# BachiLi/redner

Measured on AMD Instinct MI355X. Metric: Msamples/s fwd+bwd, higher is better.
Workload: dtype f64; 1 GPU; bunny_box 1024x1024, max_bounces 4, Sobol, 256 spp fwd+bwd per step (vertex gradients, primary+secondary edge sampling), sharded by sample index over 1 GPU(s): 256 spp per GPU; spp=256, spp_per_gpu=256, max_bounces=4, parallelism=sample-sharded x1, world_size=1, pool_cap_mb=32768, samples_per_launch=8, sample_workers=2, schedule=library default: two sample workers, batches as large as the buffer cache holds

## Files before the change

### include/redner_amd.h

```cpp
#ifndef REDNER_AMD_H
#define REDNER_AMD_H

#include <stddef.h>
#include <stdint.h>

#ifdef __cplusplus
extern "C" {
#endif

#define RDR_MAX_MIP_LEVELS 8

enum rdr_camera_type { RDR_CAMERA_PERSPECTIVE = 0, RDR_CAMERA_ORTHOGRAPHIC = 1, RDR_CAMERA_FISHEYE = 2,
                       RDR_CAMERA_PANORAMA = 3 };
enum rdr_sampler_type { RDR_SAMPLER_INDEPENDENT = 0, RDR_SAMPLER_SOBOL = 1 };
enum rdr_channel {
    RDR_CH_RADIANCE = 0, RDR_CH_ALPHA, RDR_CH_DEPTH, RDR_CH_POSITION, RDR_CH_GEOMETRY_NORMAL,
    RDR_CH_SHADING_NORMAL, RDR_CH_UV, RDR_CH_BARYCENTRIC_COORDINATES, RDR_CH_DIFFUSE_REFLECTANCE,
    RDR_CH_SPECULAR_REFLECTANCE, RDR_CH_ROUGHNESS, RDR_CH_GENERIC_TEXTURE, RDR_CH_VERTEX_COLOR,
    RDR_CH_SHAPE_ID, RDR_CH_TRIANGLE_ID, RDR_CH_MATERIAL_ID
};

typedef struct rdr_camera_desc {
    int width, height;
    const float *position, *look, *up;
// ... 58 lines not shown
    const float *env_to_world, *world_to_env;
    const float *sample_cdf_ys, *sample_cdf_xs;
    float pdf_norm;
    int directly_visible;
} rdr_envmap_desc;
typedef struct rdr_denvmap_desc { rdr_dtexture_desc values; float *world_to_env; } rdr_denvmap_desc;

typedef struct rdr_tuning rdr_tuning;
typedef struct rdr_render_options {
    uint64_t seed;
    int num_samples, max_bounces;
    const int *channels; int num_channels;
    int sampler_type;
    int sample_pixel_center;
    int sample_offset, total_samples;
    const rdr_tuning *tuning;
} rdr_render_options;

enum rdr_tune_flags {
    RDR_TUNE_NO_OVERLAP       = 1 << 0,
    RDR_TUNE_FORCE_GENERAL    = 1 << 1,
    RDR_TUNE_PICKN_WALK       = 1 << 2,
    RDR_TUNE_PICKH_FUSED      = 1 << 3,
    RDR_TUNE_PICKH_LAZY       = 1 << 4,
    RDR_TUNE_NO_HOIST         = 1 << 5,
    RDR_TUNE_REFILL_OFF       = 1 << 6,
    RDR_TUNE_REFILL_ALL       = 1 << 7,
    RDR_TUNE_TRACE_BINARY     = 1 << 8,
    RDR_TUNE_TRACE_NO_LDS_TOP = 1 << 9,
    RDR_TUNE_NO_FUSED_BOUNCE  = 1 << 10,
    RDR_TUNE_PICKH_ONE_LAUNCH = 1 << 11,
    RDR_TUNE_NO_NEE_COMPACT   = 1 << 12,
    RDR_TUNE_LARGE_FORMS      = 1 << 13,
    RDR_TUNE_TRACE_EVERY_CONTINUATION = 1 << 14
};
struct rdr_tuning {
    unsigned flags;
    int batch_samples;
    int64_t batch_lanes;
    int workers;
    int refill_rays_per_lane, refill_idle_lanes, refill_steps;
    int wide_max_rays;
    int gather_budget;
    int gather_heavy_cap_plus1, gather_work_cap_plus1;
    int mem_available_mb;
    int refill_order;
    int pickh_slots_per_lane, pickh_idle_lanes, pickh_steps;
    int stale_event_cap_plus1;
};

void rdr_set_stream(void *hip_stream);
void rdr_set_pool_cap_mb(int64_t megabytes);
int64_t rdr_get_pool_cap_mb(void);
enum rdr_build_flags {
    RDR_BUILD_NO_REFIT        = 1 << 0,
    RDR_BUILD_NO_EDGE_CACHE   = 1 << 1,
    RDR_BUILD_SYNC_EDGES      = 1 << 2,
    RDR_BUILD_EDGE_HOST_BUILD = 1 << 3
};
void rdr_set_build_flags(unsigned flags);

typedef struct rdr_dscene_desc {
    rdr_dcamera_desc camera;
    const rdr_dshape_desc *shapes; int num_shapes;
    const rdr_dmaterial_desc *materials; int num_materials;
    const rdr_darea_light_desc *area_lights; int num_area_lights;
    const rdr_denvmap_desc *envmap;
// ... 51 lines not shown
                               const float *d_normals, float *d_vertices, float *scratch, int64_t scratch_floats);

const char *rdr_last_error(void);

typedef struct rdr_trace_stats {
    double closest_ms, any_ms;
    uint64_t closest_launches, any_launches;
    uint64_t closest_rays, any_rays;
    uint64_t closest_nodes, closest_tris, any_nodes, any_tris;
    uint64_t closest_wide_nodes, any_wide_nodes;
    double closest_union_ms, any_union_ms;
} rdr_trace_stats;
void rdr_trace_stats_enable(int timing, int counting);
void rdr_trace_stats_reset(void);
void rdr_trace_stats_get(rdr_trace_stats *out);

int rdr_scene_trace(const rdr_scene *scene, const float *rays, int32_t *hits, int num_rays, int any_hit);

uint64_t rdr_trim_cache(void);

typedef struct rdr_debug_counters {
    uint64_t device_mallocs, host_count_reads;
    uint64_t last_batch_samples, last_workers;
} rdr_debug_counters;
void rdr_debug_counters_get(rdr_debug_counters *out);

int rdr_debug_bvh_check(const rdr_scene *scene);

int rdr_debug_dump_edges(const rdr_scene *scene, const char *path);

int rdr_libm_exact(void);

int rdr_debug_libm(int fn, const double *x, const double *y, double *out, int n);

#ifdef __cplusplus
}
#endif
#endif
```

### redner_amd/_capi.py

```python
import ctypes as C
import os

MAX_MIP = 8
_HERE = os.path.dirname(os.path.abspath(__file__))
DEFAULT_LIBRARY = os.path.join(_HERE, 'lib', 'libredner_amd.so')
EXACT_LIBRARY = os.path.join(_HERE, 'lib', 'libredner_amd_exact.so')

c_float_p = C.POINTER(C.c_float)
c_int_p = C.POINTER(C.c_int32)


class CameraDesc(C.Structure):
    _fields_ = [('width', C.c_int), ('height', C.c_int),
                ('position', C.c_void_p), ('look', C.c_void_p), ('up', C.c_void_p),
                ('cam_to_world', C.c_void_p), ('world_to_cam', C.c_void_p),
                ('intrinsic_mat_inv', C.c_void_p), ('intrinsic_mat', C.c_void_p),
                ('distortion_params', C.c_void_p),
                ('clip_near', C.c_float), ('camera_type', C.c_int),
                ('viewport_beg', C.c_int * 2), ('viewport_end', C.c_int * 2)]


class DCameraDesc(C.Structure):
    _fields_ = [(n, C.c_void_p) for n in ('position', 'look', 'up', 'cam_to_world', 'world_to_cam',
                                          'intrinsic_mat_inv', 'intrinsic_mat', 'distortion_params')]
# ... 31 lines not shown
                                            'generic_texture', 'normal_map')]


class AreaLightDesc(C.Structure):
    _fields_ = [('shape_id', C.c_int), ('intensity', C.c_float * 3), ('two_sided', C.c_int),
                ('directly_visible', C.c_int)]


class DAreaLightDesc(C.Structure):
    _fields_ = [('intensity', C.c_void_p)]


class EnvmapDesc(C.Structure):
    _fields_ = [('values', TextureDesc), ('env_to_world', C.c_void_p), ('world_to_env', C.c_void_p),
                ('sample_cdf_ys', C.c_void_p), ('sample_cdf_xs', C.c_void_p),
                ('pdf_norm', C.c_float), ('directly_visible', C.c_int)]


class DEnvmapDesc(C.Structure):
    _fields_ = [('values', DTextureDesc), ('world_to_env', C.c_void_p)]


class Tuning(C.Structure):
    _fields_ = [('flags', C.c_uint), ('batch_samples', C.c_int), ('batch_lanes', C.c_int64), ('workers', C.c_int),
                ('refill_rays_per_lane', C.c_int), ('refill_idle_lanes', C.c_int), ('refill_steps', C.c_int),
                ('wide_max_rays', C.c_int), ('gather_budget', C.c_int),
                ('gather_heavy_cap_plus1', C.c_int), ('gather_work_cap_plus1', C.c_int), ('mem_available_mb', C.c_int),
                ('refill_order', C.c_int), ('pickh_slots_per_lane', C.c_int), ('pickh_idle_lanes', C.c_int), ('pickh_steps', C.c_int),
                ('stale_event_cap_plus1', C.c_int)]


TUNE_NO_OVERLAP, TUNE_FORCE_GENERAL, TUNE_PICKN_WALK, TUNE_PICKH_FUSED, TUNE_PICKH_LAZY, TUNE_NO_HOIST, TUNE_REFILL_OFF, \
    TUNE_REFILL_ALL, TUNE_TRACE_BINARY, TUNE_TRACE_NO_LDS_TOP, TUNE_NO_FUSED_BOUNCE, TUNE_PICKH_ONE_LAUNCH, TUNE_NO_NEE_COMPACT, \
    TUNE_LARGE_FORMS, TUNE_TRACE_EVERY_CONTINUATION = [1 << k for k in range(15)]
BUILD_NO_REFIT, BUILD_NO_EDGE_CACHE, BUILD_SYNC_EDGES, BUILD_EDGE_HOST_BUILD = [1 << k for k in range(4)]


class RenderOptionsDesc(C.Structure):
    _fields_ = [('seed', C.c_uint64), ('num_samples', C.c_int), ('max_bounces', C.c_int),
                ('channels', C.POINTER(C.c_int)), ('num_channels', C.c_int),
                ('sampler_type', C.c_int), ('sample_pixel_center', C.c_int),
                ('sample_offset', C.c_int), ('total_samples', C.c_int),
                ('tuning', C.POINTER(Tuning))]


class DSceneDesc(C.Structure):
    _fields_ = [('camera', DCameraDesc),
                ('shapes', C.POINTER(DShapeDesc)), ('num_shapes', C.c_int),
                ('materials', C.POINTER(DMaterialDesc)), ('num_materials', C.c_int),
                ('area_lights', C.POINTER(DAreaLightDesc)), ('num_area_lights', C.c_int),
                ('envmap', C.POINTER(DEnvmapDesc))]


class TraceStats(C.Structure):
    _fields_ = [('closest_ms', C.c_double), ('any_ms', C.c_double),
                ('closest_launches', C.c_uint64), ('any_launches', C.c_uint64),
                ('closest_rays', C.c_uint64), ('any_rays', C.c_uint64),
                ('closest_nodes', C.c_uint64), ('closest_tris', C.c_uint64),
                ('any_nodes', C.c_uint64), ('any_tris', C.c_uint64),
                ('closest_wide_nodes', C.c_uint64), ('any_wide_nodes', C.c_uint64),
                ('closest_union_ms', C.c_double), ('any_union_ms', C.c_double)]


class DebugCounters(C.Structure):
    _fields_ = [('device_mallocs', C.c_uint64), ('host_count_reads', C.c_uint64),
                ('last_batch_samples', C.c_uint64), ('last_workers', C.c_uint64)]


class DeferredDesc(C.Structure):
    _fields_ = [('num_images', C.c_int), ('height', C.c_int), ('width', C.c_int),
                ('aa_samples', C.c_int), ('alpha', C.c_int), ('num_lights', C.c_int),
                ('light_type', c_int_p), ('image_light_range', c_int_p), ('gpu_index', C.c_int)]


DL_AMBIENT, DL_POINT, DL_DIRECTIONAL, DL_SPOT = range(4)

EXPORTS = ('rdr_scene_create', 'rdr_scene_destroy', 'rdr_scene_max_generic_texture_dimension',
           'rdr_render', 'rdr_compute_num_channels', 'rdr_last_error',
           'rdr_trace_stats_enable', 'rdr_trace_stats_reset', 'rdr_trace_stats_get', 'rdr_scene_trace',
           'rdr_debug_counters_get', 'rdr_trim_cache', 'rdr_debug_dump_edges', 'rdr_debug_bvh_check',
           'rdr_set_stream', 'rdr_set_pool_cap_mb', 'rdr_get_pool_cap_mb', 'rdr_set_build_flags', 'rdr_debug_libm', 'rdr_libm_exact',
           'rdr_deferred_shade', 'rdr_deferred_shade_backward',
           'rdr_mip_num_levels', 'rdr_mip_backward_scratch', 'rdr_mip_tiled_stages', 'rdr_mip_pyramid',
           'rdr_mip_pyramid_backward',
           'rdr_mesh_topology_create', 'rdr_mesh_topology_destroy', 'rdr_mesh_topology_read', 'rdr_vertex_normal_scratch',
           'rdr_vertex_normal', 'rdr_vertex_normal_backward')

_lib = None
_lib_path = None


def load(path=None):
    global _lib, _lib_path
    path = path or os.environ.get('REDNER_AMD_LIB') or \
        (EXACT_LIBRARY if os.environ.get('REDNER_AMD_LIBM', '').lower() == 'exact' else DEFAULT_LIBRARY)
    if not os.path.exists(path):
        raise RuntimeError(
            "redner_amd: native library %s not found. Build it with "
            "`python -c 'import __graft_entry__ as g; g.build()'` (hipcc, gfx950). "
            "There is no CPU fallback." % path)
    lib = C.CDLL(path)
    for name in EXPORTS:
        if not hasattr(lib, name):
            raise RuntimeError("redner_amd: %s does not export %s" % (path, name))
    lib.rdr_scene_create.restype = C.c_void_p
    lib.rdr_scene_create.argtypes = [C.POINTER(CameraDesc), C.POINTER(ShapeDesc), C.c_int,
                                     C.POINTER(MaterialDesc), C.c_int, C.POINTER(AreaLightDesc), C.c_int,
                                     C.POINTER(EnvmapDesc), C.c_int, C.c_int, C.c_int, C.c_int]
    lib.rdr_scene_destroy.restype = None
    lib.rdr_scene_destroy.argtypes = [C.c_void_p]
    lib.rdr_scene_max_generic_texture_dimension.restype = C.c_int
    lib.rdr_scene_max_generic_texture_dimension.argtypes = [C.c_void_p]
    lib.rdr_render.restype = C.c_int
    lib.rdr_render.argtypes = [C.c_void_p, C.POINTER(RenderOptionsDesc), C.c_void_p, C.c_void_p,
                               C.POINTER(DSceneDesc), C.c_void_p, C.c_void_p]
    lib.rdr_compute_num_channels.restype = C.c_int
    lib.rdr_compute_num_channels.argtypes = [C.POINTER(C.c_int), C.c_int, C.c_int]
    lib.rdr_last_error.restype = C.c_char_p
    lib.rdr_last_error.argtypes = []
    lib.rdr_trace_stats_enable.restype = None
    lib.rdr_trace_stats_enable.argtypes = [C.c_int, C.c_int]
    lib.rdr_trace_stats_reset.restype = None
    lib.rdr_debug_counters_get.restype = None
    lib.rdr_debug_counters_get.argtypes = [C.POINTER(DebugCounters)]
    lib.rdr_trim_cache.restype = C.c_uint64
    lib.rdr_trim_cache.argtypes = []
    lib.rdr_debug_bvh_check.restype = C.c_int
    lib.rdr_debug_bvh_check.argtypes = [C.c_void_p]
    lib.rdr_set_stream.restype = None
    lib.rdr_set_stream.argtypes = [C.c_void_p]
    lib.rdr_set_pool_cap_mb.restype = None
    lib.rdr_set_pool_cap_mb.argtypes = [C.c_int64]
    lib.rdr_get_pool_cap_mb.restype = C.c_int64
    lib.rdr_get_pool_cap_mb.argtypes = []
    lib.rdr_set_build_flags.restype = None
    lib.rdr_set_build_flags.argtypes = [C.c_uint]
    lib.rdr_trace_stats_get.restype = None
    lib.rdr_trace_stats_get.argtypes = [C.POINTER(TraceStats)]
    lib.rdr_scene_trace.restype = C.c_int
    lib.rdr_scene_trace.argtypes = [C.c_void_p, C.c_void_p, C.c_void_p, C.c_int, C.c_int]
    lib.rdr_libm_exact.restype = C.c_int
    lib.rdr_libm_exact.argtypes = []
    lib.rdr_debug_libm.restype = C.c_int
    lib.rdr_debug_libm.argtypes = [C.c_int, C.c_void_p, C.c_void_p, C.c_void_p, C.c_int]
    lib.rdr_deferred_shade.restype = C.c_int
    lib.rdr_deferred_shade.argtypes = [C.POINTER(DeferredDesc), C.c_void_p, C.c_void_p, C.c_void_p]
    lib.rdr_deferred_shade_backward.restype = C.c_int
    lib.rdr_deferred_shade_backward.argtypes = [C.POINTER(DeferredDesc), C.c_void_p, C.c_void_p, C.c_void_p, C.c_void_p, C.c_void_p]
    lib.rdr_mip_num_levels.restype = C.c_int
    lib.rdr_mip_num_levels.argtypes = [C.c_int, C.c_int]
    lib.rdr_mip_backward_scratch.restype = C.c_int64
    lib.rdr_mip_backward_scratch.argtypes = [C.c_int, C.c_int, C.c_int]
    lib.rdr_mip_tiled_stages.restype = C.c_int
    lib.rdr_mip_tiled_stages.argtypes = [C.c_int, C.c_int, C.c_int]
    lib.rdr_mip_pyramid.restype = C.c_int
    lib.rdr_mip_pyramid.argtypes = [C.c_int, C.c_int, C.c_int, C.c_int, C.POINTER(C.c_void_p), C.c_int]
    lib.rdr_mip_pyramid_backward.restype = C.c_int
    lib.rdr_mip_pyramid_backward.argtypes = [C.c_int, C.c_int, C.c_int, C.c_int, C.POINTER(C.c_void_p), C.c_void_p, C.c_void_p,
                                             C.c_int64, C.c_int]
    lib.rdr_mesh_topology_create.restype = C.c_void_p
    lib.rdr_mesh_topology_create.argtypes = [C.c_void_p, C.c_int, C.c_int, C.c_int, C.c_int]
    lib.rdr_mesh_topology_destroy.restype = None
    lib.rdr_mesh_topology_destroy.argtypes = [C.c_void_p]
    lib.rdr_mesh_topology_read.restype = C.c_int
    lib.rdr_mesh_topology_read.argtypes = [C.c_void_p, C.c_void_p, C.c_void_p]
    lib.rdr_vertex_normal_scratch.restype = C.c_int
    lib.rdr_vertex_normal_scratch.argtypes = [C.c_void_p, C.c_int, C.POINTER(C.c_int64), C.POINTER(C.c_int64), C.POINTER(C.c_int64)]
    lib.rdr_vertex_normal.restype = C.c_int
    lib.rdr_vertex_normal.argtypes = [C.c_void_p, C.c_int, C.c_void_p, C.c_void_p, C.c_void_p, C.c_void_p, C.c_int64]
    lib.rdr_vertex_normal_backward.restype = C.c_int
    lib.rdr_vertex_normal_backward.argtypes = [C.c_void_p, C.c_int, C.c_void_p, C.c_void_p, C.c_void_p, C.c_void_p, C.c_void_p,
                                               C.c_int64]
    _lib, _lib_path = lib, path
    return lib


def lib():
# ... 16 lines not shown
```

### redner_amd/csrc/capi.cpp

```cpp
#include "../../include/redner_amd.h"
#include "render.h"
#include "tuning.h"
#include "edges.h"
#include "deferred.h"
#include "mipmap.h"
#include "vertex_normal.h"
#include <cstdio>
#include "scene.h"
#include <cstring>
#include <exception>
#include <mutex>
#include <string>
#include <vector>
#include <cstdlib>

namespace {
thread_local std::string g_last_error;
std::recursive_mutex g_device_lock[16];
std::recursive_mutex &device_lock(int gpu_index) { return g_device_lock[(gpu_index < 0 ? 0 : gpu_index) & 15]; }
void set_error(const char *what) { g_last_error = what ? what : "unknown error"; }
thread_local void *g_user_stream = nullptr;
void use_caller_stream() { exec::ctx().stream = (hipStream_t)g_user_stream; }
}

struct LibmProbe {
    int fn; const double *x, *y; double *out;
    RDR_FN void operator()(int i) const {
        const double a = x[i], b = y[i];
        double r;
        switch (fn) {
            case 0: r = gm::sin(a); break;
            case 1: r = gm::cos(a); break;
            case 2: r = gm::atan2(a, b); break;
            case 3: r = gm::atan(a); break;
            case 4: r = gm::acos(a); break;
            case 5: r = gm::log(a); break;
            default: r = gm::pow(a, b); break;
        }
        out[i] = r;
    }
};

extern "C" {

const char *rdr_last_error(void) { return g_last_error.c_str(); }

rdr_scene *rdr_scene_create(const rdr_camera_desc *camera, const rdr_shape_desc *shapes, int num_shapes,
                            const rdr_material_desc *materials, int num_materials,
                            const rdr_area_light_desc *area_lights, int num_area_lights,
                            const rdr_envmap_desc *envmap, int use_gpu, int gpu_index,
                            int use_primary_edge_sampling, int use_secondary_edge_sampling) {
    try {
        g_last_error.clear();
        std::lock_guard<std::recursive_mutex> lk(device_lock(gpu_index));
        use_caller_stream();
        return reinterpret_cast<rdr_scene *>(rdr::create_scene(camera, shapes, num_shapes, materials, num_materials,
                                                               area_lights, num_area_lights, envmap, use_gpu, gpu_index,
                                                               use_primary_edge_sampling, use_secondary_edge_sampling));
    } catch (const std::exception &e) {
        set_error(e.what());
        return nullptr;
    }
}

void rdr_scene_destroy(rdr_scene *scene) {
    if (!scene) return;
    rdr::Scene *s = reinterpret_cast<rdr::Scene *>(scene);
    std::lock_guard<std::recursive_mutex> lk(device_lock(s->gpu_index));
    delete s;
}

int rdr_scene_max_generic_texture_dimension(const rdr_scene *scene) {
    return scene ? reinterpret_cast<const rdr::Scene *>(scene)->max_generic_texture_dimension : 0;
}
// ... 336 lines not shown
        return 0;
    } catch (const std::exception &e) {
        set_error(e.what());
        return 1;
    }
}

int rdr_debug_libm(int fn, const double *x, const double *y, double *out, int n) {
    try {
        g_last_error.clear();
        if (fn < 0 || fn > 6 || n < 0) throw std::runtime_error("rdr_debug_libm: bad arguments");
        std::lock_guard<std::recursive_mutex> lk(device_lock(exec::current_device()));
        exec::select_device(1, exec::current_device());
        use_caller_stream();
        const size_t bytes = sizeof(double) * (size_t)n;
        struct Held {
            double *p[3] = {nullptr, nullptr, nullptr};
            ~Held() { exec::device_sync(); for (double *q : p) exec::dfree(q); }
        } held;
        for (double *&q : held.p) q = (double *)exec::dmalloc(bytes);
        double *dx = held.p[0], *dy = held.p[1], *dout = held.p[2];
        exec::upload(dx, x, bytes);
        if (y) exec::upload(dy, y, bytes); else exec::zero(dy, bytes);
        exec::launch(exec::Count(n), LibmProbe{fn, dx, dy, dout});
        exec::download(out, dout, bytes);
        exec::sync();
        return 0;
    } catch (const std::exception &e) {
        set_error(e.what());
        return 1;
    }
}

}
```

### redner_amd/csrc/render.cpp

```cpp
#include "render.h"
#include "tuning.h"
#include <atomic>
#include <exception>
#include <cstdio>
#include <cstdlib>
#include "stages_fwd.h"
#include "stages_bwd.h"
#include "stages_edge.h"
#include "grad_store.h"
#include <algorithm>
#include <memory>
#include <stdexcept>
#include <type_traits>
#include <vector>

namespace rdr {

namespace {

inline bool overlap_on() { return !tuning().has(RDR_TUNE_NO_OVERLAP); }


VSlice make_slice(Arena &a, int n, bool with_occl, bool with_rdiff = true) {
    VSlice v;
// ... 152 lines not shown
    if (!fused) {
        launch_v(lean, b.num_active, contrib);
        return exec::compact_dev(b.active, b.num_active, b.next_active, KeepHit{vn.shape}, nullptr, b.dyn, b.dyn_inc);
    }
    if (b.vnn) {
        BounceSample next{sd, b.rng, b.dim + 7, b.rng_shift, b.active, vn, *b.vnn, q.nee, q.bsdf};
        next.last_bounce_emitters = b.next_is_last && emitter_test;
        launch_v(lean, b.num_active, BounceContribSample{contrib, next, qpos});
    } else if (qpos) {
        launch_v(lean, b.num_active, BounceContribSample{contrib, BounceSample{sd, b.rng, b.dim + 7, b.rng_shift, b.active, vn, vn, nullptr, nullptr}, qpos, 1});
    } else {
        launch_v(lean, b.num_active, contrib);
    }
    int *pos_out = q.pos[chain->flip];
    chain->flip ^= 1;
    const exec::Count next = exec::compact_dev(b.active, b.num_active, b.next_active, KeepHit{vn.shape}, nullptr, b.dyn, b.dyn_inc, pos_out);
    chain->have_rays = b.vnn != nullptr;
    chain->qpos = pos_out;
    chain->queue_n = b.num_active;
    return next;
}

struct BatchView { int S = 1, P0 = 0, rows = 0; bool on = false; };

struct Worker {
    Arena arena;
    std::vector<VSlice> vs;
    int *active = nullptr;
    Queues q;
    std::vector<exec::Count> num_active;
    int *main_dyn = nullptr;
    int *seg = nullptr;
    float *stage = nullptr;
    Fork shadow_fork;
};

struct Backward {
    const Scene &scene; const rdr_render_options &opt;
    Worker &w;
    int stride, B;
    const float *d_image; float *screen_grad; double weight; int nd, radiance_dim;
    BatchView batch;
    SceneD sd;
    GradStore &grads;
    Arena arena;
    AdjState adj;
    int adj_point_doubles = kAdjPointDoubles;

    ChannelsD ch;
    int lean = kGeneral;
    uint64_t *pcg_edge = nullptr;
    int *edge_dyn = nullptr;
    int *hoist_dyn = nullptr;
    double *multipliers = nullptr;

    VSlice ea, eb;
    int chain_n = 0;
    double *erd_chain = nullptr;
    int *deferred = nullptr, *deferred_seg = nullptr, *deferred_count = nullptr, *prim_dyn = nullptr;
    int *elist[3] = {nullptr, nullptr, nullptr};
    HLeaf *h_leaves = nullptr, *h_spill = nullptr;
    int *nee_act = nullptr;
    HDescent *h_descent = nullptr;
    GatherShared gshared{nullptr, nullptr, nullptr, nullptr, 0, 0};
    GatherCand *gather_cands = nullptr;
    int *nee_slots = nullptr;
// ... 270 lines not shown
        launch_v(lean, n, AdjBounceScatter{part});
    }

    void trace_edge_paths(exec::Count n_act, exec::Count n_slots, int first_depth, bool need_lights, const int *seg = nullptr, int *dyn = nullptr) {
        if (!dyn) dyn = edge_dyn;
        if (need_lights && !has_lights) return;
        int cur = 1;
        BounceChain chain;
        chain.fused = fuse_bounces(pcg_edge != nullptr, lean, n_act.upper);
        for (int depth = first_depth, k = 0; depth < B && n_act.upper > 0; ++depth, ++k) {
            const VSlice &m = (k % 2 == 0) ? ea : eb;
            const VSlice &nx = (k % 2 == 0) ? eb : ea;
            int nxt = (cur == 1) ? 2 : 1;
            Bounce b;
            b.rng = edge_rng_at(edim, dyn, seg); b.dim = edim; b.rng_shift = 1;
            b.active = elist[cur]; b.num_active = n_act; b.next_active = elist[nxt];
            b.v = &m; b.vn = &nx; b.vnn = depth + 1 < B ? &m : nullptr;
            b.q = &w.q; b.sink = esink;
            b.dyn = batch.on ? nullptr : dyn; b.dyn_inc = 7;
            b.last_bounce = depth == B - 1; b.next_is_last = depth + 2 == B;
            b.chain = &chain; b.shadow_fork = &w.shadow_fork;
            const exec::Count next = run_bounce(scene, sd, b);
            if (batch.on) exec::launch(cur_S, BumpDynList{dyn, elist[cur], n_act.dev, n_act.upper, seg, 2 * batch.P0, 7});
            edge_rng_consumed(n_slots, 7, n_act.dev);
            n_act = next;
            cur = nxt;
        }
    }

    void begin_sample(int sample_id_, const SamplerD &main_rng, int n_lanes, int S_now) {
        sample_id = sample_id_; lanes = n_lanes; cur_S = S_now;
        rng = main_rng;
        rng_edge = SamplerD{scene.sobol_table, opt.seed + 131071U, sample_id, pcg_edge, 0};
        edim = 0;
        hoisted = false;
        if (edge_dyn) exec::zero(edge_dyn, sizeof(int) * kMaxBatch);
        if (chain_mode()) exec::zero(ea.erd_touched, (size_t)ea.n);
        if (hp_written) exec::zero(hp_written, (size_t)ea.n);
        clear_adjoint_records();
        if (adj.carries) exec::zero(adj.carries, (size_t)stride);
    }

    void sweep_depth(int d) {
        const exec::Count nA = w.num_active[d];
        if (nA.upper <= 0) return;
        const AdjBounceArgs ba{sd, grads.g, rng, dim0 + 7 * d, active_of(d), w.vs[d], w.vs[d + 1], d_image, nd, radiance_dim, weight, adj};
        bool with_edges = secondary_on();
        if (with_edges && d > 0 && scene.diffuse_only) {
            with_edges = false;
            secondary_pass_consumed(nA, d);
        }
        const bool early_here = hoisted && d == 0;
        const bool side = overlap && with_edges && !early_here;
        beside(adjoint_fork, side, 0, lanes, [&] {
            adj_scatter(ba, nA, d);
            adj_nee(ba, nA, d);
        });
        if (with_edges) secondary_edge_pass(d, nA, early_here, side);
    }
    void secondary_edge_pass(int d, exec::Count nA, bool early_here, bool side) {
        const exec::Count edge_lanes = exec::scaled_count(nA, 2);
        if (chain_mode()) erd_view(seg_of(d));
        const SecEdgeArgs sa = early_here ? early_sa : start_picks(d, edim, nullptr, false, side);
        join_picks();
        debug_dump("sec_mode", sample_id, d, sec_mode, (size_t)nA.upper);
        debug_dump("sec_picks", sample_id, d, sec_picks, sizeof(SecPick) * (size_t)nA.upper);
// ... 193 lines not shown
    const bool samples_independent = batchable && d_image != nullptr && image == nullptr;
    const bool forward_batches = sobol_plain && d_image == nullptr && image != nullptr;
    const BatchView batch = choose_batch(opt, tune, P, cam.vp_y1 - cam.vp_y0, lean, lay.nd, samples_independent, forward_batches, d_image != nullptr);
    const int S = batch.S;
    const int PL = S * P;
    static const bool tell = std::getenv("RDR_DEBUG_BATCH") != nullptr;
    if (tell) std::fprintf(stderr, "[render] %s: %d samples of %d lanes in batches of %d\n", d_image ? "backward" : "forward", opt.num_samples, P, S);
    const int num_batches = (opt.num_samples + S - 1) / S;
    const float *d_image_lanes = d_image;
    if (batch.on && d_image) {
        float *rep = arena.get<float>((size_t)PL * lay.nd);
        for (int k = 0; k < S; ++k)
            exec::copy_dev(rep + (size_t)k * P * lay.nd, d_image, sizeof(float) * (size_t)P * lay.nd);
        d_image_lanes = rep;
    }
    const int *assign_flags = batch.on && forward_batches && !lay.ch.radiance_only ? upload_assign_flags(arena, opt, scene.max_generic_texture_dimension, lay.nd) : nullptr;
    int workers = 1;
    if (samples_independent) workers = std::max(1, std::min(tune.workers > 0 ? tune.workers : exec::sample_workers(PL, num_batches, batch.on), num_batches));
    if (chain) workers = 1;
    if (d_image != nullptr) { last_schedule()[0].store(S); last_schedule()[1].store(workers); }

    struct SampleWorker : Worker { std::unique_ptr<Backward> bwd; };
    auto make_worker = [&](SampleWorker &w) {
        w.vs.resize(B + 1);
        for (int d = 0; d <= B; ++d) w.vs[d] = make_slice(w.arena, PL, d < B && d_image_lanes != nullptr, lean != kLean);
        w.active = w.arena.get<int>((size_t)(B + 1) * PL);
        w.q.nee = w.arena.get<rt::RayRec>((size_t)2 * PL); w.q.bsdf = w.arena.get<rt::RayRec>((size_t)2 * PL);
        w.q.h_nee = w.arena.get<rt::HitRec>((size_t)2 * PL); w.q.h_bsdf = w.arena.get<rt::HitRec>((size_t)2 * PL);
        w.q.pos[0] = w.arena.get<int>((size_t)2 * PL); w.q.pos[1] = w.arena.get<int>((size_t)2 * PL);
        w.num_active.assign(B + 2, exec::Count(0));
        if (pcg_main) w.main_dyn = w.arena.get<int>(1);
        if (batch.on) w.seg = w.arena.get<int>((size_t)(B + 1) * (kMaxBatch + 1));
        if (batch.on && forward_batches) w.stage = w.arena.get<float>((size_t)(B + 1) * PL * lay.nd);
    };
    auto run_samples = [&](SampleWorker &w, int first, int stride) {
        std::vector<VSlice> &vs = w.vs;
        int *active = w.active;
        const Queues &q = w.q;
        std::vector<exec::Count> &num_active = w.num_active;
        SceneD sd = scene.d;
        if (batch.on) sd.cam.batch_rows = batch.rows;
        for (int b = first; b < num_batches; b += stride) {
            const int s = b * S;
            const int S_now = std::min(S, opt.num_samples - s);
            const int lanes = S_now * P;
            const int sample_id = opt.sample_offset + s;
            SamplerD rng{scene.sobol_table, opt.seed, sample_id, pcg_main, 0};
            if (batch.on) { rng.batch = S_now; rng.batch_lanes = P; }
            Sink sink{image, nullptr, lay.nd, lay.radiance_dim, weight, lay.ch, nullptr};
            const size_t plane = (size_t)PL * lay.nd;
            auto sink_of = [&](int launch) { Sink k = sink; if (w.stage) k.image = w.stage + (size_t)launch * plane; return k; };
            if (w.stage) exec::zero(w.stage, sizeof(float) * plane * (B + 1));
            auto segments = [&](int d) {
                if (batch.on) exec::launch(S_now + 1, SegOffsets{active + (size_t)d * PL, num_active[d].dev, num_active[d].upper, P, S_now,
                                                                 w.seg + (size_t)d * (kMaxBatch + 1)});
            };

            launch_v(lean, lanes, GenPrimary{sd, rng, opt.sample_pixel_center, vs[0], q.bsdf});
            exec::trace(scene.bvh, q.bsdf, q.h_bsdf, lanes, false, true);
            launch_v(lean, lanes, ShadePrimary{sd, nullptr, vs[0], q.h_bsdf, sink_of(0)});
            std::fill(num_active.begin(), num_active.end(), exec::Count(0));
            num_active[0] = exec::compact_dev((const int *)nullptr, lanes, active, KeepHit{vs[0].shape});
            if (d_image) segments(0);
            if (w.main_dyn) exec::zero(w.main_dyn, sizeof(int));

            int dim = opt.sample_pixel_center ? 0 : 2;
            const int dim_first = dim;
            BounceChain chain;
            chain.fused = fuse_bounces(pcg_main != nullptr, lean, 2 * lanes);
            for (int d = 0; d < B && num_active[d].upper > 0 && has_lights; ++d) {
                Bounce bounce;
                bounce.rng = rng; bounce.dim = dim;
                bounce.active = active + (size_t)d * PL; bounce.num_active = num_active[d]; bounce.next_active = active + (size_t)(d + 1) * PL;
                bounce.v = &vs[d]; bounce.vn = &vs[d + 1]; bounce.vnn = d + 1 < B ? &vs[d + 2] : nullptr;
                bounce.q = &q; bounce.sink = sink_of(d + 1);
                bounce.dyn = w.main_dyn; bounce.dyn_inc = 7;
                bounce.shadow_rays_coherent = d == 0;
                bounce.last_bounce = d == B - 1; bounce.next_is_last = d + 2 == B;
                bounce.chain = &chain; bounce.shadow_fork = &w.shadow_fork;
                num_active[d + 1] = run_bounce(scene, sd, bounce);
                if (num_active[d + 1].dev && d_image) segments(d + 1);
// ... 76 lines not shown
```

### redner_amd/csrc/sobol.h

```cpp
#pragma once
#include <stdint.h>

namespace rdr {

constexpr int kSobolBits = 52;
constexpr int kSamplerDims = 1024;
constexpr int kSobolTableWords = kSobolBits * kSamplerDims;

RDR_FN uint64_t hash64shift(uint64_t key) {
    key = (~key) + (key << 21);
    key = key ^ (key >> 24);
    key = (key + (key << 3)) + (key << 8);
    key = key ^ (key >> 14);
    key = (key + (key << 2)) + (key << 4);
    key = key ^ (key >> 28);
    key = key + (key << 31);
    return key;
}

RDR_FN uint64_t sobol_scramble(uint64_t seed, int slot) { return hash64shift((seed << 32) | (uint64_t)slot); }

RDR_FN double sobol_value(const uint64_t *matrices, uint64_t index, uint32_t dim, uint64_t scramble) {
    uint64_t r = scramble & ~-(1ULL << kSobolBits);
    const uint64_t *m = matrices + (size_t)dim * kSobolBits;
// ... 13 lines not shown
    uint64_t inc = pcg_inc(slot);
    uint64_t st = pcg_step(0U, inc);
    st += (0x853c49e6748fea9bULL + seed);
    return pcg_step(st, inc);
}
RDR_FN uint64_t pcg_advance(uint64_t state, uint64_t inc, uint32_t delta) {
    uint64_t acc_mult = 1, acc_plus = 0, cur_mult = kPcgMult, cur_plus = inc | 1;
    while (delta > 0) {
        if (delta & 1) { acc_mult *= cur_mult; acc_plus = acc_plus * cur_mult + cur_plus; }
        cur_plus = (cur_mult + 1) * cur_plus;
        cur_mult *= cur_mult;
        delta >>= 1;
    }
    return acc_mult * state + acc_plus;
}
RDR_FN double pcg_output_double(uint64_t oldstate) {
    uint32_t xorshifted = uint32_t(((oldstate >> 18u) ^ oldstate) >> 27u);
    uint32_t rot = uint32_t(oldstate >> 59u);
    uint32_t u = uint32_t((xorshifted >> rot) | (xorshifted << ((-rot) & 31)));
    union { uint64_t u; double d; } x;
    x.u = ((uint64_t)u << 20) | 0x3ff0000000000000ULL;
    return x.d - 1.0;
}

struct SamplerD {
    const uint64_t *matrices;
    uint64_t seed;
    int sample_id;
    const uint64_t *pcg_state;
    int pcg_base;
    const int *dyn = nullptr;
    int batch = 0, batch_lanes = 0;
    const int *seg = nullptr;
    struct Lane { uint64_t index, scramble; int slot, dyn; };
    RDR_FN Lane lane(int slot) const {
        Lane l;
        l.slot = slot; l.index = 0; l.scramble = 0; l.dyn = 0;
        if (pcg_state) return l;
        int s = 0;
        if (seg) {
            for (int k = 1; k < batch; ++k) if (slot >= seg[k]) s = k;
            slot -= seg[s];
        } else if (batch_lanes > 0) {
            s = slot / batch_lanes;
            slot -= s * batch_lanes;
        }
        l.index = (uint64_t)(sample_id + s);
        l.scramble = sobol_scramble(seed, slot);
        l.dyn = dyn ? dyn[s] : 0;
        return l;
    }
    RDR_FN double draw(const Lane &l, int dim) const {
        if (pcg_state) return pcg_output_double(pcg_advance(pcg_state[l.slot], pcg_inc(l.slot), (uint32_t)(dim - pcg_base)));
        return sobol_value(matrices, l.index, (uint32_t)(dim + l.dyn), l.scramble);
    }
    RDR_FN double draw(int slot, int dim) const { return draw(lane(slot), dim); }
};

struct PcgInit {
    uint64_t *state; uint64_t seed;
    RDR_FN void operator()(int slot) const { state[slot] = pcg_seed_state(seed, slot); }
};
struct PcgAdvance {
    uint64_t *state; int count;
    const int *extra = nullptr, *gate = nullptr;
    RDR_FN void operator()(int slot) const {
        if (gate && *gate <= 0) return;
        state[slot] = pcg_advance(state[slot], pcg_inc(slot), (uint32_t)(count + (extra ? *extra : 0)));
    }
};

struct BumpDyn {
    int *dyn; const int *gate; int inc;
    RDR_FN void operator()(int) const { if (!gate || *gate > 0) *dyn += inc; }
};
constexpr int kDepthGates = 16;
struct CountLiveDepths {
    int *out; const int *gate[kDepthGates]; int n, inc, add;
    RDR_FN void operator()(int) const {
        int c = add ? *out : 0;
        for (int i = 0; i < kDepthGates; ++i) if (i < n && *gate[i] > 0) c += inc;
        *out = c;
    }
};

constexpr int kMaxBatch = 16;
struct SegOffsets {
    const int *list; const int *count; int upper, lanes_per_sample, batch; int *out;
    RDR_FN void operator()(int s) const {
// ... 56 lines not shown
```

### redner_amd/csrc/tuning.h

```cpp
#pragma once
#include "../../include/redner_amd.h"
#include <atomic>
#include <cstdio>
#include <cstdlib>

namespace rdr {

struct Tuning {
    unsigned flags = 0;
    int batch_samples = 16;
    long long batch_lanes = 0;
    int workers = 0;
    int refill_k = 4, refill_idle = 24, refill_steps = 4;
    int wide_max = 1 << 19;
    int gather_budget = 256;
    int gather_heavy_cap = -1, gather_work_cap = -1;
    double mem_available_mb = -1.0;
    int refill_sort = 1;
    int pickh_k = 1, pickh_idle = 8, pickh_steps = 8;
    int stale_event_cap = -1;
    bool has(unsigned f) const { return (flags & f) != 0; }
};

namespace detail {
inline const char *env(const char *name) { return std::getenv(name); }
inline bool env_set(const char *name) { return std::getenv(name) != nullptr; }
struct EnvDefaults {
    unsigned flags = 0;
    int batch_samples = 0; long long batch_lanes = 0; int workers = 0;
    int refill_k = 0, refill_idle = 0, refill_steps = 0, wide_max = 0, gather_budget = 0, heavy_cap = -1, work_cap = -1;
    double mem_mb = -1.0;
    int refill_order = 0, pickh_k = 0, pickh_idle = 0, pickh_steps = 0;
    EnvDefaults() {
        if (env_set("RDR_NO_OVERLAP") || env_set("RDR_DEBUG_DUMP")) flags |= RDR_TUNE_NO_OVERLAP;
        if (env_set("RDR_FORCE_GENERAL")) flags |= RDR_TUNE_FORCE_GENERAL;
        if (env_set("RDR_PICKN_WALK")) flags |= RDR_TUNE_PICKN_WALK;
        if (env_set("RDR_PICKH_FUSED")) flags |= RDR_TUNE_PICKH_FUSED;
        if (env_set("RDR_PICKH_LAZY")) flags |= RDR_TUNE_PICKH_LAZY;
        if (env_set("RDR_NO_HOIST")) flags |= RDR_TUNE_NO_HOIST;
        if (env_set("RDR_TRACE_REFILL_ALL")) flags |= RDR_TUNE_REFILL_ALL;
        if (env_set("RDR_TRACE_BINARY")) flags |= RDR_TUNE_TRACE_BINARY;
        if (env_set("RDR_TRACE_NO_LDS_TOP")) flags |= RDR_TUNE_TRACE_NO_LDS_TOP;
        if (env_set("RDR_NO_FUSED_BOUNCE")) flags |= RDR_TUNE_NO_FUSED_BOUNCE;
        if (env_set("RDR_PICKH_ONE_LAUNCH")) flags |= RDR_TUNE_PICKH_ONE_LAUNCH;
        if (env_set("RDR_NO_NEE_COMPACT")) flags |= RDR_TUNE_NO_NEE_COMPACT;
        if (env_set("RDR_LARGE_FRAME_FORMS")) flags |= RDR_TUNE_LARGE_FORMS;
        if (env_set("RDR_TRACE_EVERY_CONTINUATION")) flags |= RDR_TUNE_TRACE_EVERY_CONTINUATION;
        if (const char *e = env("RDR_TRACE_REFILL")) {
            int k = 0, idle = 0, steps = 0;
            const int got = std::sscanf(e, "%d,%d,%d", &k, &idle, &steps);
            if (got >= 1 && k <= 0) flags |= RDR_TUNE_REFILL_OFF;
            if (got >= 1 && k > 0) refill_k = k;
            if (got >= 2 && idle > 0) refill_idle = idle;
            if (got >= 3 && steps > 0) refill_steps = steps;
        }
        if (const char *e = env("RDR_BATCH")) batch_samples = std::atoi(e);
        if (const char *e = env("RDR_BATCH_LANES")) batch_lanes = std::atoll(e);
        if (const char *e = env("RDR_WORKERS")) workers = std::atoi(e);
        if (const char *e = env("RDR_WIDE_MAX")) wide_max = std::atoi(e);
        if (const char *e = env("RDR_GATHER_BUDGET")) gather_budget = std::atoi(e);
        if (const char *e = env("RDR_GATHER_CAPS")) { int h = 0, w = 0; if (std::sscanf(e, "%d,%d", &h, &w) == 2) { heavy_cap = h; work_cap = w; } }
        if (const char *e = env("RDR_MEM_AVAILABLE_MB")) mem_mb = std::atof(e);
        if (const char *e = env("RDR_REFILL_SORT")) refill_order = std::atoi(e) + 1;
        if (const char *e = env("RDR_PICKH_REFILL")) {
            int k = 0, idle = 0, steps = 0;
            const int got = std::sscanf(e, "%d,%d,%d", &k, &idle, &steps);
            if (got >= 1 && k > 0) pickh_k = k;
            if (got >= 2 && idle > 0) pickh_idle = idle;
            if (got >= 3 && steps > 0) pickh_steps = steps;
        }
    }
};
inline const EnvDefaults &env_defaults() { static const EnvDefaults d; return d; }
inline int clampi(long long v, long long lo, long long hi) { return (int)(v < lo ? lo : (v > hi ? hi : v)); }
}

inline Tuning resolve_tuning(const rdr_tuning *t) {
    const detail::EnvDefaults &e = detail::env_defaults();
    static const rdr_tuning zero{};
    const rdr_tuning &u = t ? *t : zero;
// ... 47 lines not shown
```

Measured before the change: 85.87 Msamples/s.

## Precompute per-sample Sobol matrix products once per batch and reuse across lanes

Adds a SobolRows kernel that computes the Sobol generator-matrix XOR product once per (sample, dimension) for the current batch into a small device table. Each lane's draw then becomes a scramble XOR with the table entry instead of a per-lane loop over matrix bits. The intent is to remove redundant Sobol index computation repeated for every pixel lane. In exchange it adds an extra small launch per batch and a global table read per draw. The old per-lane path stays available behind a flag, and a debug probe compares the two paths.

```diff
diff --git a/include/redner_amd.h b/include/redner_amd.h
--- a/include/redner_amd.h
+++ b/include/redner_amd.h
@@ -114,7 +114,8 @@
     RDR_TUNE_PICKH_ONE_LAUNCH = 1 << 11,
     RDR_TUNE_NO_NEE_COMPACT   = 1 << 12,
     RDR_TUNE_LARGE_FORMS      = 1 << 13,
-    RDR_TUNE_TRACE_EVERY_CONTINUATION = 1 << 14
+    RDR_TUNE_TRACE_EVERY_CONTINUATION = 1 << 14,
+    RDR_TUNE_SOBOL_PER_LANE   = 1 << 15
 };
 struct rdr_tuning {
     unsigned flags;
@@ -232,6 +233,8 @@
 int rdr_libm_exact(void);
 
 int rdr_debug_libm(int fn, const double *x, const double *y, double *out, int n);
+int rdr_debug_sobol(const int64_t *sample_index, const int *dim, const int *slot, int n, uint64_t seed,
+                    int64_t first_index, int rows, double *out_table, double *out_per_lane);
 
 #ifdef __cplusplus
 }
diff --git a/redner_amd/_capi.py b/redner_amd/_capi.py
--- a/redner_amd/_capi.py
+++ b/redner_amd/_capi.py
@@ -87,7 +87,7 @@
 
 TUNE_NO_OVERLAP, TUNE_FORCE_GENERAL, TUNE_PICKN_WALK, TUNE_PICKH_FUSED, TUNE_PICKH_LAZY, TUNE_NO_HOIST, TUNE_REFILL_OFF, \
     TUNE_REFILL_ALL, TUNE_TRACE_BINARY, TUNE_TRACE_NO_LDS_TOP, TUNE_NO_FUSED_BOUNCE, TUNE_PICKH_ONE_LAUNCH, TUNE_NO_NEE_COMPACT, \
-    TUNE_LARGE_FORMS, TUNE_TRACE_EVERY_CONTINUATION = [1 << k for k in range(15)]
+    TUNE_LARGE_FORMS, TUNE_TRACE_EVERY_CONTINUATION, TUNE_SOBOL_PER_LANE = [1 << k for k in range(16)]
 BUILD_NO_REFIT, BUILD_NO_EDGE_CACHE, BUILD_SYNC_EDGES, BUILD_EDGE_HOST_BUILD = [1 << k for k in range(4)]
 
 
@@ -134,7 +134,8 @@
            'rdr_render', 'rdr_compute_num_channels', 'rdr_last_error',
            'rdr_trace_stats_enable', 'rdr_trace_stats_reset', 'rdr_trace_stats_get', 'rdr_scene_trace',
            'rdr_debug_counters_get', 'rdr_trim_cache', 'rdr_debug_dump_edges', 'rdr_debug_bvh_check',
-           'rdr_set_stream', 'rdr_set_pool_cap_mb', 'rdr_get_pool_cap_mb', 'rdr_set_build_flags', 'rdr_debug_libm', 'rdr_libm_exact',
+           'rdr_set_stream', 'rdr_set_pool_cap_mb', 'rdr_get_pool_cap_mb', 'rdr_set_build_flags', 'rdr_debug_libm', 'rdr_debug_sobol',
+           'rdr_libm_exact',
            'rdr_deferred_shade', 'rdr_deferred_shade_backward',
            'rdr_mip_num_levels', 'rdr_mip_backward_scratch', 'rdr_mip_tiled_stages', 'rdr_mip_pyramid',
            'rdr_mip_pyramid_backward',
@@ -198,6 +199,9 @@
     lib.rdr_libm_exact.argtypes = []
     lib.rdr_debug_libm.restype = C.c_int
     lib.rdr_debug_libm.argtypes = [C.c_int, C.c_void_p, C.c_void_p, C.c_void_p, C.c_int]
+    lib.rdr_debug_sobol.restype = C.c_int
+    lib.rdr_debug_sobol.argtypes = [C.c_void_p, C.c_void_p, C.c_void_p, C.c_int, C.c_uint64, C.c_int64, C.c_int,
+                                    C.c_void_p, C.c_void_p]
     lib.rdr_deferred_shade.restype = C.c_int
     lib.rdr_deferred_shade.argtypes = [C.POINTER(DeferredDesc), C.c_void_p, C.c_void_p, C.c_void_p]
     lib.rdr_deferred_shade_backward.restype = C.c_int
diff --git a/redner_amd/csrc/capi.cpp b/redner_amd/csrc/capi.cpp
--- a/redner_amd/csrc/capi.cpp
+++ b/redner_amd/csrc/capi.cpp
@@ -5,6 +5,8 @@
 #include "deferred.h"
 #include "mipmap.h"
 #include "vertex_normal.h"
+#include "sobol.h"
+#include <cstdint>
 #include <cstdio>
 #include "scene.h"
 #include <cstring>
@@ -40,6 +42,16 @@
         out[i] = r;
     }
 };
+
+constexpr int kSobolProbeLanes = 1 << 26;
+struct SobolProbe {
+    rdr::SamplerD rng; const int64_t *sample; const int *dim, *slot; double *out;
+    RDR_FN void operator()(int i) const {
+        const int s = (int)(sample[i] - (int64_t)rng.sample_id);
+        out[i] = rng.draw(s * kSobolProbeLanes + slot[i], dim[i]);
+    }
+};
+extern "C" const uint64_t rdr_sobol_table[];
 
 extern "C" {
 
@@ -442,4 +454,49 @@
     }
 }
 
-}
+int rdr_debug_sobol(const int64_t *sample_index, const int *dim, const int *slot, int n, uint64_t seed,
+                    int64_t first_index, int rows, double *out_table, double *out_per_lane) {
+    try {
+        g_last_error.clear();
+        if (n < 0 || rows < 1 || rows > rdr::kMaxBatch || first_index < 0 || first_index + rows - 1 > INT32_MAX)
+            throw std::runtime_error("rdr_debug_sobol: bad arguments");
+        for (int i = 0; i < n; ++i)
+            if (sample_index[i] < first_index || sample_index[i] >= first_index + rows || dim[i] < 0 || dim[i] >= rdr::kSamplerDims ||
+                slot[i] < 0 || slot[i] >= kSobolProbeLanes)
+                throw std::runtime_error("rdr_debug_sobol: a number lies outside the table");
+        std::lock_guard<std::recursive_mutex> lk(device_lock(exec::current_device()));
+        exec::select_device(1, exec::current_device());
+        use_caller_stream();
+        const size_t count = (size_t)(n > 0 ? n : 1);
+        const size_t sizes[6] = {sizeof(int64_t) * count, sizeof(int) * count, sizeof(int) * count, sizeof(double) * count,
+                                 sizeof(double) * count, sizeof(uint64_t) * (size_t)rdr::kMaxBatch * rdr::kSamplerDims};
+        struct Held {
+            void *p[6] = {nullptr, nullptr, nullptr, nullptr, nullptr, nullptr};
+            ~Held() { exec::device_sync(); for (void *q : p) exec::dfree(q); }
+        } held;
+        for (int k = 0; k < 6; ++k) held.p[k] = exec::dmalloc(sizes[k]);
+        int64_t *d_sample = (int64_t *)held.p[0];
+        int *d_dim = (int *)held.p[1], *d_slot = (int *)held.p[2];
+        double *d_table_out = (double *)held.p[3], *d_lane_out = (double *)held.p[4];
+        uint64_t *d_rows = (uint64_t *)held.p[5];
+        exec::upload(d_sample, sample_index, sizeof(int64_t) * (size_t)n);
+        exec::upload(d_dim, dim, sizeof(int) * (size_t)n);
+        exec::upload(d_slot, slot, sizeof(int) * (size_t)n);
+        const uint64_t *matrices = (const uint64_t *)exec::device_constant(rdr_sobol_table, sizeof(uint64_t) * (size_t)rdr::kSobolTableWords);
+        exec::launch(exec::Count(rows * rdr::kSamplerDims), rdr::SobolRows{matrices, (uint64_t)first_index, rows, d_rows});
+        rdr::SamplerD rng{matrices, seed, (int)first_index, nullptr, 0};
+        rng.batch = rows; rng.batch_lanes = kSobolProbeLanes;
+        exec::launch(exec::Count(n), SobolProbe{rng, d_sample, d_dim, d_slot, d_lane_out});
+        rng.pre = d_rows;
+        exec::launch(exec::Count(n), SobolProbe{rng, d_sample, d_dim, d_slot, d_table_out});
+        exec::download(out_per_lane, d_lane_out, sizeof(double) * (size_t)n);
+        exec::download(out_table, d_table_out, sizeof(double) * (size_t)n);
+        exec::sync();
+        return 0;
+    } catch (const std::exception &e) {
+        set_error(e.what());
+        return 1;
+    }
+}
+
+}
diff --git a/redner_amd/csrc/render.cpp b/redner_amd/csrc/render.cpp
--- a/redner_amd/csrc/render.cpp
+++ b/redner_amd/csrc/render.cpp
@@ -208,6 +208,7 @@
     int *main_dyn = nullptr;
     int *seg = nullptr;
     float *stage = nullptr;
+    uint64_t *sobol_rows = nullptr;
     Fork shadow_fork;
 };
 
@@ -544,6 +545,7 @@
         sample_id = sample_id_; lanes = n_lanes; cur_S = S_now;
         rng = main_rng;
         rng_edge = SamplerD{scene.sobol_table, opt.seed + 131071U, sample_id, pcg_edge, 0};
+        rng_edge.pre = main_rng.pre;
         edim = 0;
         hoisted = false;
         if (edge_dyn) exec::zero(edge_dyn, sizeof(int) * kMaxBatch);
@@ -803,6 +805,7 @@
         if (pcg_main) w.main_dyn = w.arena.get<int>(1);
         if (batch.on) w.seg = w.arena.get<int>((size_t)(B + 1) * (kMaxBatch + 1));
         if (batch.on && forward_batches) w.stage = w.arena.get<float>((size_t)(B + 1) * PL * lay.nd);
+        if (!pcg_main && !tune.has(RDR_TUNE_SOBOL_PER_LANE)) w.sobol_rows = w.arena.get<uint64_t>((size_t)kMaxBatch * kSamplerDims);
     };
     auto run_samples = [&](SampleWorker &w, int first, int stride) {
         std::vector<VSlice> &vs = w.vs;
@@ -818,6 +821,10 @@
             const int sample_id = opt.sample_offset + s;
             SamplerD rng{scene.sobol_table, opt.seed, sample_id, pcg_main, 0};
             if (batch.on) { rng.batch = S_now; rng.batch_lanes = P; }
+            if (w.sobol_rows) {
+                exec::launch(S_now * kSamplerDims, SobolRows{scene.sobol_table, (uint64_t)sample_id, S_now, w.sobol_rows});
+                rng.pre = w.sobol_rows;
+            }
             Sink sink{image, nullptr, lay.nd, lay.radiance_dim, weight, lay.ch, nullptr};
             const size_t plane = (size_t)PL * lay.nd;
             auto sink_of = [&](int launch) { Sink k = sink; if (w.stage) k.image = w.stage + (size_t)launch * plane; return k; };
diff --git a/redner_amd/csrc/sobol.h b/redner_amd/csrc/sobol.h
--- a/redner_amd/csrc/sobol.h
+++ b/redner_amd/csrc/sobol.h
@@ -69,10 +69,11 @@
     const int *dyn = nullptr;
     int batch = 0, batch_lanes = 0;
     const int *seg = nullptr;
-    struct Lane { uint64_t index, scramble; int slot, dyn; };
+    const uint64_t *pre = nullptr;
+    struct Lane { uint64_t scramble; int slot, row, s; };
     RDR_FN Lane lane(int slot) const {
         Lane l;
-        l.slot = slot; l.index = 0; l.scramble = 0; l.dyn = 0;
+        l.slot = slot; l.scramble = 0; l.row = 0; l.s = 0;
         if (pcg_state) return l;
         int s = 0;
         if (seg) {
@@ -82,16 +83,31 @@
             s = slot / batch_lanes;
             slot -= s * batch_lanes;
         }
-        l.index = (uint64_t)(sample_id + s);
+        l.s = s;
         l.scramble = sobol_scramble(seed, slot);
-        l.dyn = dyn ? dyn[s] : 0;
+        l.row = (pre ? s * kSamplerDims : 0) + (dyn ? dyn[s] : 0);
         return l;
     }
     RDR_FN double draw(const Lane &l, int dim) const {
         if (pcg_state) return pcg_output_double(pcg_advance(pcg_state[l.slot], pcg_inc(l.slot), (uint32_t)(dim - pcg_base)));
-        return sobol_value(matrices, l.index, (uint32_t)(dim + l.dyn), l.scramble);
+        if (pre) return ((l.scramble & ~-(1ULL << kSobolBits)) ^ pre[l.row + dim]) * (1.0 / (1ULL << kSobolBits));
+        return sobol_value(matrices, (uint64_t)(sample_id + l.s), (uint32_t)(dim + l.row), l.scramble);
     }
     RDR_FN double draw(int slot, int dim) const { return draw(lane(slot), dim); }
+};
+
+struct SobolRows {
+    const uint64_t *matrices; uint64_t first_index; int rows; uint64_t *out;
+    RDR_FN void operator()(int i) const {
+        const int s = i / kSamplerDims, dim = i - s * kSamplerDims;
+        if (s >= rows) return;
+        const uint64_t *m = matrices + (size_t)dim * kSobolBits;
+        uint64_t r = 0;
+        uint64_t index = first_index + (uint64_t)s;
+        for (int k = 0; index && k < kSobolBits; index >>= 1, ++k)
+            if (index & 1) r ^= m[k];
+        out[i] = r;
+    }
 };
 
 struct PcgInit {
diff --git a/redner_amd/csrc/tuning.h b/redner_amd/csrc/tuning.h
--- a/redner_amd/csrc/tuning.h
+++ b/redner_amd/csrc/tuning.h
@@ -46,6 +46,7 @@
         if (env_set("RDR_NO_NEE_COMPACT")) flags |= RDR_TUNE_NO_NEE_COMPACT;
         if (env_set("RDR_LARGE_FRAME_FORMS")) flags |= RDR_TUNE_LARGE_FORMS;
         if (env_set("RDR_TRACE_EVERY_CONTINUATION")) flags |= RDR_TUNE_TRACE_EVERY_CONTINUATION;
+        if (env_set("RDR_SOBOL_PER_LANE")) flags |= RDR_TUNE_SOBOL_PER_LANE;
         if (const char *e = env("RDR_TRACE_REFILL")) {
             int k = 0, idle = 0, steps = 0;
             const int got = std::sscanf(e, "%d,%d,%d", &k, &idle, &steps);
```

Result: no change. 86.46 Msamples/s (median of 6 runs) (+0.7%).
